# libnxz/power-gzip

Measured on AMD Instinct MI355X. Metric: GiB/s uncompressed in (deflate), real-data corpus in 64 KiB blocks, exact dynamic-Huffman table per block, higher is better.
Workload: dtype u8

## Files before the change

### power-gzip_amd/csrc/nxz_lz77.hip

```cpp
#include <hip/hip_runtime.h>
#include <type_traits>
#include <stdint.h>
#include "nxz_device.h"
#include "nxz_dhtgen_dev.h"
#include "nxz_dict.h"

__device__ unsigned long long *nxz_lz77_prof_buf = nullptr;
#define NXZ_GLOBAL NXZ_GLOBAL_AS
#ifdef NXZ_LZ77_PROF
#define WPROF_BEGIN() unsigned long long wp_ = prof ? clock64() : 0
#define WPROF_END(idx) do { if (prof) { const unsigned long long now_ = clock64(); wacc[(idx) - 16] += now_ - wp_; wp_ = now_; } } while (0)
#define PROF(idx) do { if (prof) { if (t == 0) { unsigned long long now_ = clock64(); profacc[idx] += (uint32_t)(now_ - tprev); tprev = now_; } } } while (0)
#define PCOUNT(idx, n) do { if (prof && lane == 0) atomicAdd(&profacc[idx], (uint32_t)(n)); } while (0)
#ifdef NXZ_LZ77_PROF2
#define PC2(idx, n) do { if (prof && lane == 0) __hip_atomic_fetch_add(&prof[32 + (idx)], (unsigned long long)(n), __ATOMIC_RELAXED, __HIP_MEMORY_SCOPE_AGENT); } while (0)
#else
#define PC2(idx, n) do { } while (0)
#endif
#else
#define PC2(idx, n) do { } while (0)
#define PCOUNT(idx, n) do { } while (0)
#define WPROF_BEGIN() do { } while (0)
#define WPROF_END(idx) do { } while (0)
#define PROF(idx) do { } while (0)
#endif

namespace nxzl77 {

constexpr int NT = 1024;
constexpr int HBITS = 13;
constexpr uint32_t HSIZE = 1u << HBITS;
constexpr uint32_t PTILE = 16384;
constexpr uint32_t PSEG = 16;
constexpr uint32_t NSEG = PTILE / PSEG;
constexpr uint32_t ETILE = 2048;
constexpr uint32_t LAZY_MAX = 32;
constexpr uint32_t MAXMATCH = 258;
constexpr uint32_t WINDOW = 32768;
constexpr uint32_t OPEN2 = 24;
constexpr uint32_t NOHASH = 0xFFFFu;
constexpr uint32_t SECOND_MIN_TOKENS = 3072;
constexpr uint32_t TEXT_HIGH_DIV = 16;
#ifndef NXZ_GROUP_ROUNDS
#define NXZ_GROUP_ROUNDS 24
#endif
#ifndef NXZ_GROUP_MIN
#define NXZ_GROUP_MIN 2
#endif
#ifndef NXZ_GROUP_GATE
#define NXZ_GROUP_GATE 3
#endif
constexpr uint32_t GROUP_ROUNDS = NXZ_GROUP_ROUNDS;
constexpr uint32_t GROUP_GATE = NXZ_GROUP_GATE;
constexpr uint32_t GROUP_MIN = NXZ_GROUP_MIN;
constexpr uint32_t C2_STRIDE = PTILE + 1024;

constexpr uint32_t OFF_IN    = 0;
constexpr uint32_t OFF_HEAD  = 65536 + 32;
constexpr uint32_t OFF_CAND  = OFF_HEAD + HSIZE * 4 + 256;
constexpr uint32_t OFF_MLEN  = OFF_CAND + PTILE * 2;
constexpr uint32_t OFF_SBITS = OFF_MLEN + PTILE;
constexpr uint32_t OFF_MBITS = OFF_SBITS + PTILE / 8;
constexpr uint32_t OFF_X     = OFF_MBITS + PTILE / 8;
constexpr uint32_t OFF_ENTRY = OFF_X + NSEG * 2;
constexpr uint32_t OFF_BITS  = OFF_ENTRY + NSEG * 2;
#ifndef NXZ_LQ_CAP
#define NXZ_LQ_CAP 128
#define NXZ_LQ_MIN 64
#endif
#ifndef NXZ_XQ_CAP
#define NXZ_XQ_CAP 120
#define NXZ_XQ_MIN 56
#endif
constexpr uint32_t LQ_CAP = NXZ_LQ_CAP, LQ_MIN = NXZ_LQ_MIN, XQ_CAP = NXZ_XQ_CAP, XQ_MIN = NXZ_XQ_MIN;
static_assert(LQ_MIN + 64 <= LQ_CAP && XQ_MIN + 64 <= XQ_CAP && LQ_CAP % 8 == 0 && XQ_CAP % 8 == 0, "a batch of 64 must fit behind what waits");
constexpr uint32_t BITS_BYTES = 16 * (LQ_CAP + XQ_CAP) * 2 + 2096 - NSEG * 4 < ETILE * 2 + 64 ? ETILE * 2 + 64 : 16 * (LQ_CAP + XQ_CAP) * 2 + 2096 - NSEG * 4;
constexpr uint32_t OFF_LQ    = OFF_X;
constexpr uint32_t OFF_DQ    = OFF_LQ;
constexpr uint32_t OFF_XQ    = OFF_LQ + 16 * LQ_CAP * 2;
constexpr uint32_t OFF_EB    = OFF_XQ + 16 * XQ_CAP * 2;
constexpr uint32_t EBO       = 32;
static_assert(OFF_EB % 16 == 0 && OFF_EB + 2096 <= OFF_BITS + BITS_BYTES, "match-phase carve");
constexpr uint32_t OFF_SCAN  = OFF_BITS + BITS_BYTES;
constexpr uint32_t OFF_HIST  = OFF_SCAN + 256;
constexpr uint32_t OFF_MISC  = OFF_HIST + 316 * 4;
constexpr uint32_t OFF_PROF  = OFF_MISC + 64;
constexpr uint32_t LDS_BYTES = OFF_PROF + 80;
static_assert(LDS_BYTES <= 163840, "LDS budget");
static_assert(OFF_HEAD % 16 == 0 && OFF_BITS % 16 == 0 && OFF_SCAN % 16 == 0, "alignment");

enum { M_NREC = 0, M_TOK0 = 1, M_HIGH = 2, M_DQ = 3, M_PROGRESS = 4, M_TICKET = 5, M_DEFER = 6, M_NEXT = 7, M_KEEP = 8, M_DEFER2 = 9, M_PREV = 12, M_JOBNO = 13 };
static_assert(M_TICKET == M_PROGRESS + 1 && M_DEFER == M_PROGRESS + 2, "cleared together");

__device__ __forceinline__ uint32_t lds_ld32(const uint32_t *inw, uint32_t r)
{
	uint32_t a = inw[r >> 2], b = inw[(r >> 2) + 1];
	return __builtin_amdgcn_alignbyte(b, a, r & 3);
}

__device__ __forceinline__ uint32_t hash4(uint32_t v) { return (v * 0x9E3779B1u) >> (32 - HBITS); }

__device__ __forceinline__ uint32_t equal16(const uint32_t *inw, uint32_t a, uint32_t b)
{
	const uint32_t aw = a >> 2, bw = b >> 2, as = a & 3, bs = b & 3;
	const uint32_t a0 = inw[aw], a1 = inw[aw + 1], a2 = inw[aw + 2], a3 = inw[aw + 3], a4 = inw[aw + 4];
	const uint32_t b0 = inw[bw], b1 = inw[bw + 1], b2 = inw[bw + 2], b3 = inw[bw + 3], b4 = inw[bw + 4];
	const uint32_t x0 = __builtin_amdgcn_alignbyte(a1, a0, as) ^ __builtin_amdgcn_alignbyte(b1, b0, bs);
	const uint32_t x1 = __builtin_amdgcn_alignbyte(a2, a1, as) ^ __builtin_amdgcn_alignbyte(b2, b1, bs);
	const uint32_t x2 = __builtin_amdgcn_alignbyte(a3, a2, as) ^ __builtin_amdgcn_alignbyte(b3, b2, bs);
	const uint32_t x3 = __builtin_amdgcn_alignbyte(a4, a3, as) ^ __builtin_amdgcn_alignbyte(b4, b3, bs);
	uint32_t n = 16;
	if (x3) n = 12 + ((uint32_t)__builtin_ctz(x3) >> 3);
	if (x2) n = 8 + ((uint32_t)__builtin_ctz(x2) >> 3);
	if (x1) n = 4 + ((uint32_t)__builtin_ctz(x1) >> 3);
	if (x0) n = (uint32_t)__builtin_ctz(x0) >> 3;
	return n;
}

__device__ __forceinline__ uint32_t gf_mul(uint32_t a, uint32_t b)
{
	uint32_t r = 0;
#pragma unroll 8
	for (int i = 0; i < 32; i++) {
		r ^= (b & 0x80000000u) ? a : 0;
// ... 393 lines not shown
					  uint8_t *__restrict__ tokens, uint16_t *__restrict__ cand2,
					  nxz_batch_result_t *__restrict__ results,
					  uint32_t *__restrict__ counts, uint32_t njobs, uint32_t *__restrict__ next_job,
					  const uint8_t *__restrict__ dict)
{
	__shared__ __attribute__((aligned(16))) uint8_t lds[LDS_BYTES];
	uint32_t *inw = (uint32_t *)(lds + OFF_IN);
	uint32_t *head = (uint32_t *)(lds + OFF_HEAD);
	uint16_t *cand = (uint16_t *)(lds + OFF_CAND);
	uint8_t *mlen = lds + OFF_MLEN;
	uint16_t *X = (uint16_t *)(lds + OFF_X);
	uint16_t *entry = (uint16_t *)(lds + OFF_ENTRY);
	uint32_t *sbits = (uint32_t *)(lds + OFF_SBITS);
	uint32_t *mbits = (uint32_t *)(lds + OFF_MBITS);
	uint32_t *tokbits = sbits;
	uint32_t *litbits = mbits;
	uint8_t *mark = lds + OFF_SBITS;
	uint16_t *jump = (uint16_t *)(lds + OFF_MBITS);
	uint32_t *bitbuf = (uint32_t *)(lds + OFF_BITS);
	uint32_t *scan = (uint32_t *)(lds + OFF_SCAN);
	uint32_t *hist = (uint32_t *)(lds + OFF_HIST);
	uint32_t *misc = (uint32_t *)(lds + OFF_MISC);
#ifdef NXZ_LZ77_PROF
	uint32_t *profacc = (uint32_t *)(lds + OFF_PROF);
#endif

#ifdef NXZ_LZ77_PROF
	NXZ_GLOBAL unsigned long long *prof = (NXZ_GLOBAL unsigned long long *)nxz_lz77_prof_buf;
#endif
	if constexpr (GEN) {
		if (threadIdx.x == 0) { misc[M_PREV] = 0; misc[M_JOBNO] = 0; }
		__syncthreads();
	}
	for (uint32_t bid = blockIdx.x; bid < njobs;) {
	if (next_job && threadIdx.x == 0) misc[M_NEXT] = gridDim.x + atomicAdd(next_job, 1u);
	int tid_ = threadIdx.x;
	asm volatile("" : "+v"(tid_));
	const int t = tid_, lane = t & 63, wave = t >> 6;
#ifdef NXZ_LZ77_PROF
	unsigned long long tprev = prof ? clock64() : 0;
	unsigned long long wacc[4] = { 0, 0, 0, 0 };
#endif
	const nxz_batch_job_t job = jobs[bid];
	const uint32_t total = job.src_len;
	const uint32_t h = job.hist_len < total ? job.hist_len : total;
	const uint32_t n = total - h;
	const uint32_t end = total;
	const NXZ_GLOBAL uint8_t *src = (const NXZ_GLOBAL uint8_t *)job.src;
	const uint32_t K1 = n ? (end - 1) >> 6 : 0;
	const uint32_t pw_slice = CRC_POW.v[(1022 - t) & 1023];
	const uint32_t pw_tail = CRC_POW8.v[n ? end - K1 * 64 : 0];

	{
		typedef uint32_t v4u __attribute__((ext_vector_type(4)));
		const NXZ_GLOBAL v4u *s4 = (const NXZ_GLOBAL v4u *)src;
		v4u *d4 = (v4u *)inw;
		uint32_t nfull = total >> 4;
		if constexpr (DICT) {
			const NXZ_GLOBAL v4u *w4 = (const NXZ_GLOBAL v4u *)dict;
			const uint32_t hq = h >> 4;
			for (uint32_t i = t; i < nfull; i += NT) d4[i] = i < hq ? w4[i] : s4[i];
		} else
		for (uint32_t i = t; i < nfull; i += NT) d4[i] = s4[i];
		uint32_t base = nfull << 4;
		for (uint32_t i = base + t; i < base + 48 && i < 65536 + 32; i += NT)
			lds[OFF_IN + i] = i < total ? src[i] : 0;
	}
	for (uint32_t i = t; i < HSIZE; i += NT) head[i] = 0;
	if (t < 316) hist[t] = 0;
	if (t < 16 && t != M_NEXT && !(GEN && (t == M_PREV || t == M_JOBNO))) misc[t] = FUSED && t == M_KEEP ? 3u : 0u;
#ifdef NXZ_LZ77_PROF
	if (t < 20) profacc[t] = 0;
#endif
	{
		uint32_t c = t & 255;
		for (int k = 0; k < 8 * ((t >> 8) + 1); k++) c = (c >> 1) ^ ((c & 1) ? 0xedb88320u : 0);
		bitbuf[t] = c;
	}
	__syncthreads();
	PROF(0);

	uint32_t out_crc, out_adler;
	{
		uint32_t *T = bitbuf;
		const uint32_t initx = job.in_crc ^ 0xffffffffu;
		const int sidx = (int)t - 1023 + (int)K1;
		uint32_t crc = 0, s1 = 0, sj = 0;
		if (n && sidx >= (int)(h >> 6)) {
			const uint4 *sp = (const uint4 *)(lds + OFF_IN + (uint32_t)sidx * 64);
			uint4 q[4] = { sp[0], sp[1], sp[2], sp[3] };
			uint32_t *w = (uint32_t *)q;
			const uint32_t a0 = (uint32_t)sidx * 64;
			if (a0 < h || a0 + 64 > end) {
#pragma unroll
				for (int k = 0; k < 16; k++)
					if (a0 + 4 * k < h || a0 + 4 * k + 4 > end) w[k] = 0;
			}
			uint32_t S = 0, Wt = 0;
#pragma unroll
			for (int k = 0; k < 16; k++) {
				S = __builtin_amdgcn_udot4(w[k], 0x01010101u, S, false);
				Wt = __builtin_amdgcn_udot4(w[k], 0x03020100u + 0x04040404u * k, Wt, false);
			}
			s1 = S;
			sj = S * (n + h - a0) - Wt;
			const uint32_t kfirst = a0 < h ? (h - a0) >> 2 : 0;
			if (a0 <= h && h < a0 + 64) {
				if (h + 4 <= end) {
					if (kfirst == 0) w[0] ^= initx;
					if (kfirst == 4) w[4] ^= initx;
					if (kfirst == 8) w[8] ^= initx;
					if (kfirst == 12) w[12] ^= initx;
				}
			}
			const uint32_t nd = a0 + 64 <= end ? 16 : (end - a0) >> 2;
// ... 9 lines not shown
				uint32_t b0 = v & 0xff, b1 = (v >> 8) & 0xff, b2 = (v >> 16) & 0xff;
				s1 += b0 + b1 + b2;
				sj += (b0 + b1 + b2) * (n - i) - (b1 + 2 * b2);
				if (i == 0) crc ^= initx;
				for (uint32_t k = 0; k < nb; k++) crc = T[(crc ^ (v >> (8 * k))) & 0xff] ^ (crc >> 8);
			}
		}
		uint32_t tailcrc = 0;
		if (t == 1023) { tailcrc = crc; crc = 0; }
		else if (crc) crc = gf_mul(crc, pw_slice);
		for (int o = 32; o > 0; o >>= 1) crc ^= __shfl_down(crc, o, 64);
		if (lane == 0) scan[wave] = crc;
		if (t == 1023) scan[50] = tailcrc;
		uint32_t a1 = s1, a2 = sj % 65521u;
		for (int o = 32; o > 0; o >>= 1) {
			a1 += __shfl_down(a1, o, 64);
			a2 += __shfl_down(a2, o, 64);
		}
		if (lane == 0) { scan[16 + wave] = a1; scan[32 + wave] = a2 % 65521u; }
		__syncthreads();
		if (wave == 0) {
			uint32_t c = lane < 16 ? scan[lane] : 0;
			uint32_t b1 = lane < 16 ? scan[16 + lane] : 0, b2 = lane < 16 ? scan[32 + lane] : 0;
			for (int o = 8; o > 0; o >>= 1) {
				c ^= __shfl_down(c, o, 64);
				b1 += __shfl_down(b1, o, 64);
				b2 += __shfl_down(b2, o, 64);
			}
			if (lane == 0) {
				c = n ? gf_mul(c, pw_tail) ^ scan[50] : initx;
				uint32_t ia = job.in_adler & 0xffff, ib = job.in_adler >> 16;
				uint32_t s1f = (ia + b1) % 65521u;
				uint32_t s2f = (uint32_t)(((uint64_t)ib + (uint64_t)n * ia + b2) % 65521u);
				scan[48] = c ^ 0xffffffffu;
				scan[49] = (s2f << 16) | s1f;
			}
		}
		__syncthreads();
		out_crc = __builtin_amdgcn_readfirstlane(scan[48]);
		out_adler = __builtin_amdgcn_readfirstlane(scan[49]);
		__syncthreads();
	}
	PROF(1);

	if (h) {
		uint32_t *top = (uint32_t *)cand;
		for (uint32_t i = t; i < HSIZE; i += NT) top[i] = 0;
		__syncthreads();
		for (uint32_t r = t; r < h; r += NT)
			if (r + 4 <= end) {
				const uint32_t v = lds_ld32(inw, r);
				const bool deep = r >= 8 && lds_ld32(inw, r - 8) == v && lds_ld32(inw, r - 4) == v && v == __builtin_amdgcn_alignbyte(v, v, 1);
				if (!deep) atomicMax(&top[hash4(v)], r + 1);
			}
		__syncthreads();
		for (uint32_t r = t; r < h; r += NT)
			if (r + 4 <= end) {
				const uint32_t v = lds_ld32(inw, r);
				const bool deep = r >= 8 && lds_ld32(inw, r - 8) == v && lds_ld32(inw, r - 4) == v && v == __builtin_amdgcn_alignbyte(v, v, 1);
				if (!deep && top[hash4(v)] != r + 1) atomicMax(&head[hash4(v)], r + 1);
			}
		__syncthreads();
		for (uint32_t i = t; i < HSIZE; i += NT) head[i] = top[i] | (head[i] << 16);
	}

	NXZ_GLOBAL uint32_t *dstw = (NXZ_GLOBAL uint32_t *)job.dst;
	const uint32_t cap_words = job.dst_cap >> 2;
	uint32_t wordbase = 0, obits = 3;
	const uint32_t gslot = GEN ? (uint32_t)__builtin_amdgcn_readfirstlane((int)misc[M_JOBNO]) & 1u : 0u;
	NXZ_GLOBAL uint8_t *tk = (NXZ_GLOBAL uint8_t *)tokens + (GEN ? ((size_t)blockIdx.x * 2 + gslot) : (size_t)bid) * NXZ_TOK_STRIDE;
	NXZ_GLOBAL uint32_t *g_lit = (NXZ_GLOBAL uint32_t *)(tk + NXZ_TOK_LITBITS);
	NXZ_GLOBAL uint32_t *g_tok = (NXZ_GLOBAL uint32_t *)(tk + NXZ_TOK_MATCHBITS);
	NXZ_GLOBAL uint32_t *g_rec = (NXZ_GLOBAL uint32_t *)(tk + NXZ_TOK_RECORDS);
	NXZ_GLOBAL uint16_t *g_c2 = (NXZ_GLOBAL uint16_t *)cand2 + (size_t)blockIdx.x * C2_STRIDE;
	__syncthreads();

	PROF(2);

	for (uint32_t tb0 = 0; tb0 < n; tb0 += PTILE) {
		const uint32_t tn = n - tb0 < PTILE ? n - tb0 : PTILE;
		const uint32_t nseg = (tn + PSEG - 1) / PSEG;
		const bool hard = __builtin_amdgcn_readfirstlane(misc[M_TOK0]) >= SECOND_MIN_TOKENS;
		const bool text = __builtin_amdgcn_readfirstlane(misc[M_HIGH]) * TEXT_HIGH_DIV < (n < PTILE ? n : PTILE);
		const bool use2 = tb0 == 0 || (hard && !text);
		const uint32_t lazy_max = tb0 != 0 && hard && text ? 0u : LAZY_MAX;
#ifdef NXZ_CHAIN_ALWAYS2
#define CHAIN_USE2 true
#else
#define CHAIN_USE2 use2
#endif

		const uint32_t tnpad = (tn + 511) & ~511u;
		const uint32_t npieces = tnpad >> 9;
		if (t < 3) misc[M_PROGRESS + t] = 0;
		if (t == 3) misc[M_DEFER2] = 0;
		if (t == 4) misc[M_DQ] = 0;
		sbits[t] = 0;
		uint32_t nhigh = 0;
		for (uint32_t piece = wave; piece < npieces; piece += NT / 64) {
#pragma unroll
			for (int it = 0; it < 2; it++) {
				const uint32_t i = (piece << 9) + (it << 8) + 4 * lane, r = h + tb0 + i;
				const uint32_t d0 = inw[r >> 2], d1 = inw[(r >> 2) + 1];
				if (tb0 == 0 && i < tn) nhigh += (uint32_t)__popc(d0 & 0x80808080u);
				const uint32_t v1 = __builtin_amdgcn_alignbyte(d1, d0, 1), v2 = __builtin_amdgcn_alignbyte(d1, d0, 2), v3 = __builtin_amdgcn_alignbyte(d1, d0, 3);
				uint32_t o0 = hash4(d0) << 2, o1 = hash4(v1) << 2, o2 = hash4(v2) << 2, o3 = hash4(v3) << 2;
				const uint32_t dummy = (HSIZE + ((4 * lane) & 63)) * 4;
				if (i + 4 > tn || r + 7 > end) {
					if (i + 0 >= tn || r + 4 > end) o0 = dummy;
					if (i + 1 >= tn || r + 5 > end) o1 = dummy + 4;
					if (i + 2 >= tn || r + 6 > end) o2 = dummy + 8;
					if (i + 3 >= tn || r + 7 > end) o3 = dummy + 12;
				}
				if (r >= 8 && d0 == __builtin_amdgcn_alignbyte(d0, d0, 1) && inw[(r >> 2) - 1] == d0) {
					const uint32_t x2 = inw[(r >> 2) - 2] ^ d0, y = d1 ^ d0;
					if (x2 == 0) o0 = dummy;
					if ((x2 & 0xffffff00u) == 0 && (y & 0xffu) == 0) o1 = dummy + 4;
					if ((x2 & 0xffff0000u) == 0 && (y & 0xffffu) == 0) o2 = dummy + 8;
					if ((x2 & 0xff000000u) == 0 && (y & 0xffffffu) == 0) o3 = dummy + 12;
				}
				*(uint2 *)(cand + i) = make_uint2(o0 | o1 << 16, o2 | o3 << 16);
			}
			__builtin_amdgcn_wave_barrier();
			uint32_t o[8];
#pragma unroll
			for (int u = 0; u < 8; u++) o[u] = cand[(piece << 9) + (u << 6) + lane];
			__builtin_amdgcn_wave_barrier();
			((uint4 *)cand)[(piece << 6) + lane] = make_uint4(o[0] | o[1] << 16, o[2] | o[3] << 16, o[4] | o[5] << 16, o[6] | o[7] << 16);
		}
		if (tb0 == 0) {
			for (int o = 32; o > 0; o >>= 1) nhigh += __shfl_down(nhigh, o, 64);
			if (lane == 0 && nhigh) atomicAdd(&misc[M_HIGH], nhigh);
		}
		{
			uint16_t *eb16 = (uint16_t *)(lds + OFF_EB);
			const uint32_t ngroups = (tn + EBO + 288 + 15) / 16 + 2;
			for (uint32_t g = t; g < ngroups; g += NT) {
				const int32_t r0s = (int32_t)(h + tb0 + 16 * g) - (int32_t)EBO;
				const uint32_t r0 = r0s < 0 ? end : (uint32_t)r0s;
				uint32_t bits = 0;
				if (r0 < end) {
					const uint4 dv = *(const uint4 *)(lds + OFF_IN + r0);
					const uint32_t pv = r0 ? inw[(r0 >> 2) - 1] : 0;
					auto eq4 = [](uint32_t d, uint32_t prev) -> uint32_t {
						const uint32_t xx = d ^ __builtin_amdgcn_alignbyte(d, prev, 3);
						const uint32_t nzb = (((xx & 0x7f7f7f7fu) + 0x7f7f7f7fu) | xx) & 0x80808080u;
						return ~((((nzb >> 7) * 0x00204081u) >> 21)) & 0xf;
					};
					bits = eq4(dv.x, pv) | eq4(dv.y, dv.x) << 4 | eq4(dv.z, dv.y) << 8 | eq4(dv.w, dv.z) << 12;
					if (r0 == 0) bits &= ~1u;
					if (end - r0 < 16) bits &= (1u << (end - r0)) - 1;
				}
				eb16[g] = (uint16_t)bits;
			}
		}
		__syncthreads();
		PROF(3);

		if (wave == 0) {
			uint8_t *headb = (uint8_t *)head;
			__builtin_amdgcn_s_setprio(3);
			int clane = lane;
			asm volatile("" : "+v"(clane));
			auto unpack = [](const uint4 pk, uint32_t (&off)[8]) {
				off[0] = pk.x & 0xffff; off[1] = pk.x >> 16; off[2] = pk.y & 0xffff; off[3] = pk.y >> 16;
				off[4] = pk.z & 0xffff; off[5] = pk.z >> 16; off[6] = pk.w & 0xffff; off[7] = pk.w >> 16;
			};
			auto steps = [&](const uint4 pk, uint32_t piece, uint32_t (&old)[8]) {
				uint32_t off[8]; unpack(pk, off);
#pragma unroll
				for (int u = 0; u < 8; u++) {
					uint32_t *slot = (uint32_t *)(headb + off[u]);
					old[u] = __hip_atomic_load(slot, __ATOMIC_RELAXED, __HIP_MEMORY_SCOPE_WORKGROUP);
					__builtin_amdgcn_wave_barrier();
					*(uint16_t *)slot = (uint16_t)(h + tb0 + (piece << 9) + 64 * u + clane + 1);
					__builtin_amdgcn_wave_barrier();
				}
			};
			auto note = [&](const uint4 pk, const uint32_t (&old)[8]) {
				if (!CHAIN_USE2) return;
				uint32_t off[8]; unpack(pk, off);
#pragma unroll
				for (int u = 0; u < 8; u++) *(uint16_t *)(headb + off[u] + 2) = (uint16_t)old[u];
				__builtin_amdgcn_wave_barrier();
			};
			auto hand = [&](const uint32_t (&o)[8], uint32_t piece) {
				typedef uint32_t v4u __attribute__((ext_vector_type(4)));
#pragma unroll
				for (int u = 0; u < 8; u++) cand[(piece << 9) + 64 * u + lane] = (uint16_t)o[u];
				if (CHAIN_USE2) {
					((NXZ_GLOBAL v4u *)g_c2)[(piece << 6) + lane] = (v4u){ __builtin_amdgcn_perm(o[1], o[0], 0x07060302), __builtin_amdgcn_perm(o[3], o[2], 0x07060302),
											    __builtin_amdgcn_perm(o[5], o[4], 0x07060302), __builtin_amdgcn_perm(o[7], o[6], 0x07060302) };
					__builtin_amdgcn_wave_barrier();
					__builtin_amdgcn_s_waitcnt(0x0F71);
				}
				__builtin_amdgcn_wave_barrier();
				if (lane == 0) __hip_atomic_store(&misc[M_PROGRESS], piece, __ATOMIC_RELAXED, __HIP_MEMORY_SCOPE_WORKGROUP);
				__builtin_amdgcn_wave_barrier();
			};
			const uint32_t dm = (HSIZE + lane) * 4 | ((HSIZE + lane) * 4) << 16;
			const uint4 dummy = make_uint4(dm, dm, dm, dm);
			uint4 pkB = dummy;
			uint32_t oA[8], oB[8];
			for (uint32_t base = 0; base < npieces; base += 2) {
				const uint4 *cp = (const uint4 *)cand + (base << 6) + lane;
				const bool two = base + 1 < npieces;
				const uint4 l1 = cp[two ? 64 : 0];
				const uint4 pkA = cp[0];
				steps(pkA, base, oA);
				if (base) { note(pkB, oB); hand(oB, base - 1); }
				pkB = two ? l1 : dummy;
				steps(pkB, base + 1, oB);
				note(pkA, oA);
				hand(oA, base);
			}
			{
				const uint32_t lastp = ((npieces + 1) & ~1u) - 1;
				note(pkB, oB);
				hand(oB, lastp);
				__builtin_amdgcn_s_waitcnt(0x0F70);
				__builtin_amdgcn_wave_barrier();
				if (lane == 0) __hip_atomic_store(&misc[M_PROGRESS], npieces, __ATOMIC_RELAXED, __HIP_MEMORY_SCOPE_WORKGROUP);
			}
			__builtin_amdgcn_s_setprio(0);
		}
		PROF(4);

		auto first_zero = [](const uint32_t *bm, uint32_t s0, uint32_t limit) -> uint32_t {
			uint32_t wi = (s0 >> 5) & ~3u;
			uint4 q = *(const uint4 *)(bm + wi);
			const uint32_t sw = (s0 >> 5) & 3, lowmask = ~(~0u << (s0 & 31));
			uint32_t w0 = ~q.x, w1 = ~q.y, w2 = ~q.z, w3 = ~q.w;
			if (sw > 0) w0 = 0; if (sw > 1) w1 = 0; if (sw > 2) w2 = 0;
			if (sw == 0) w0 &= ~lowmask; else if (sw == 1) w1 &= ~lowmask; else if (sw == 2) w2 &= ~lowmask; else w3 &= ~lowmask;
			for (;;) {
				if (w0 | w1 | w2 | w3) {
					const uint32_t pos = wi * 32 + (w0 ? (uint32_t)__builtin_ctz(w0) : w1 ? 32 + (uint32_t)__builtin_ctz(w1)
								  : w2 ? 64 + (uint32_t)__builtin_ctz(w2) : 96 + (uint32_t)__builtin_ctz(w3));
					return pos < limit ? pos : limit;
				}
				wi += 4;
				if (wi * 32 >= limit) return limit;
				q = *(const uint4 *)(bm + wi);
				w0 = ~q.x; w1 = ~q.y; w2 = ~q.z; w3 = ~q.w;
			}
		};
		uint32_t *kb = mbits;
		uint32_t *vb = sbits;
		{
			const uint32_t *eb = (const uint32_t *)(lds + OFF_EB);
			auto bits32 = [](const uint32_t *bm, uint32_t b) -> uint32_t {
				const uint32_t lo = bm[b >> 5], hi = bm[(b >> 5) + 1], sh = b & 31;
				return sh ? (lo >> sh) | (hi << (32 - sh)) : lo;
			};
			uint16_t *lq = (uint16_t *)(lds + OFF_LQ) + wave * LQ_CAP;
// ... 150 lines not shown
					}
					const unsigned long long ml = __ballot(open);
					if (ml) {
						if (open) xq[xqn + __popcll(ml & ((1ull << lane) - 1))] = (uint16_t)i;
						xqn += (uint32_t)__popcll(ml);
						PCOUNT(14, __popcll(ml));
						__builtin_amdgcn_wave_barrier();
					}
					pb &= pb - 1;
					const bool more = __ballot(pb != 0) != 0;
					if (xqn >= XQ_MIN || (last && !more && nq <= 64 && xqn)) { level2(xqn); xqn = 0; }
					if (!more) break;
				} while (true);
			};
			const uint32_t nunits = (tn + 255) >> 8;
			for (;;) {
				uint32_t unit = 0;
				if (lane == 0) unit = atomicAdd(&misc[M_TICKET], 1u);
				unit = __builtin_amdgcn_readfirstlane(unit);
				const bool last = unit >= nunits;
				const uint32_t piece = unit >> 1;
				uint32_t qbits = 0;
				const uint32_t it = unit & 1;
				const uint32_t ib = unit << 8;
				const uint32_t i4 = ib + 4 * lane, r4 = h + tb0 + i4;
				WPROF_BEGIN();
				if (!last) {
					while (__hip_atomic_load(&misc[M_PROGRESS], __ATOMIC_RELAXED, __HIP_MEMORY_SCOPE_WORKGROUP) <= piece)
						__builtin_amdgcn_s_sleep(4);
					__builtin_amdgcn_fence(__ATOMIC_ACQUIRE, "workgroup");
					WPROF_END(16);
					auto quad = [&](auto fullt, auto use2t) {
						constexpr bool FULL = decltype(fullt)::value, USE2 = decltype(use2t)::value;
						uint32_t q2[4] = { 0, 0, 0, 0 };
						if constexpr (USE2) {
#pragma unroll
							for (int j = 0; j < 4; j++)
								q2[j] = __hip_atomic_load(g_c2 + (piece << 9) + (4 * (lane & 15) + j) * 8 + 4 * it + (lane >> 4), __ATOMIC_RELAXED, __HIP_MEMORY_SCOPE_AGENT);
						}
						const uint2 qq = *(const uint2 *)(cand + i4);
						const uint32_t w14 = bits32(eb, EBO + i4 - 7);
						const uint32_t d0 = inw[r4 >> 2], d1 = inw[(r4 >> 2) + 1], d2 = inw[(r4 >> 2) + 2];
						uint32_t mw = 0, c01 = 0, c23 = 0, vbits = 0, kbits = 0;
						bool okA[4], raw8[4], lng[4];
						uint32_t dA[4];
#pragma unroll
						for (int j = 0; j < 4; j++) {
							const uint32_t i = i4 + j, r = r4 + j;
							const bool ok = (FULL || (i < tn && r + 4 <= end)) && ((w14 >> j) & 0x7ff) != 0x7ff;
							const uint32_t maxlen = FULL || end - r >= MAXMATCH ? MAXMATCH : end - r;
							const uint32_t v = j ? __builtin_amdgcn_alignbyte(d1, d0, j) : d0, v4 = j ? __builtin_amdgcn_alignbyte(d2, d1, j) : d1;
							auto probe = [&](uint32_t entry, uint32_t &dist1) -> uint32_t {
								const uint32_t qc = (uint16_t)(entry - 1);
								dist1 = r - qc - 1;
								const bool qok = ok && dist1 < WINDOW;
								const uint32_t q = FULL || qok ? qc : 0;
								const uint32_t qa = q >> 2, u0 = inw[qa], u1 = inw[qa + 1], u2 = inw[qa + 2];
								const uint32_t qv = __builtin_amdgcn_alignbyte(u1, u0, q & 3), qv4 = __builtin_amdgcn_alignbyte(u2, u1, q & 3);
								const uint32_t x = qv4 ^ v4;
								uint32_t n8 = 4 + ((x ? (uint32_t)__builtin_ctz(x) : 32u) >> 3);
								if (!FULL && n8 > maxlen) n8 = maxlen;
								return qok && qv == v ? n8 : 0;
							};
							uint32_t d1st, d2nd;
							const uint32_t n1st = probe((j & 2 ? qq.y : qq.x) >> (16 * (j & 1)), d1st);
							uint32_t n2nd = 0;
							d2nd = 0;
							if constexpr (USE2) n2nd = probe(q2[j], d2nd);
							const bool second = n2nd > n1st;
							const uint32_t lenA = second ? n2nd : n1st;
							okA[j] = lenA != 0;
							dA[j] = second ? d2nd : d1st;
							raw8[j] = lenA == 8;
// ... 291 lines not shown
					}
					break;
				}
				const uint32_t rest = (seg_nz | vis1) >> k;
				uint32_t run = rest ? (uint32_t)__builtin_ctz(rest) : 16 - k;
				if (run > lim - p) run = lim - p;
				if (run) {
					lm |= ((1u << run) - 1) << k;
					p += run;
					continue;
				}
				bool m;
				const uint32_t l = seg_step(p, lim, m);
				lm |= (m ? 0u : 1u) << k;
				mm |= (m ? 1u : 0u) << k;
				if (m) mlen[p] = (uint8_t)(l - 3);
				p += l;
			}
			const uint32_t sh = 16 * ((uint32_t)t & 1), wi = (uint32_t)t >> 1;
			const uint64_t lv = (uint64_t)lm << sh, mv = (uint64_t)mm << sh;
			if ((uint32_t)lv) atomicOr(&litbits[wi], (uint32_t)lv);
			if (lv >> 32) atomicOr(&litbits[wi + 1], (uint32_t)(lv >> 32));
			if ((uint32_t)mv) atomicOr(&tokbits[wi], (uint32_t)mv);
			if (mv >> 32) atomicOr(&tokbits[wi + 1], (uint32_t)(mv >> 32));
		}
		__syncthreads();
		PROF(8);
		if (tb0 == 0 && n > PTILE && t < 512) {
			uint32_t c = (uint32_t)__popc(litbits[t]) + (uint32_t)__popc(tokbits[t]);
			for (int o = 32; o > 0; o >>= 1) c += __shfl_down(c, o, 64);
			if (lane == 0) atomicAdd(&misc[M_TOK0], c);
		}

		if constexpr (FUSED) {
			Quad q[4] = { {0, 0, 0, 0}, {0, 0, 0, 0}, {0, 0, 0, 0}, {0, 0, 0, 0} };
			uint32_t nb = 0;
			if (p0 < tn) {
				const uint32_t tok16 = ((const uint16_t *)tokbits)[t], lit16 = ((const uint16_t *)litbits)[t];
				if (tok16 | lit16) {
					const uint4 bv = *(const uint4 *)(lds + OFF_IN + h + tb0 + p0);
					const uint4 mv = *(const uint4 *)(mlen + p0);
					const uint4 c0 = ((const uint4 *)cand)[2 * t], c1 = ((const uint4 *)cand)[2 * t + 1];
					q[0] = fx_quad(bv.x, lit16 & 15, tok16 & 15, mv.x, c0.x, c0.y);
					q[1] = fx_quad(bv.y, (lit16 >> 4) & 15, (tok16 >> 4) & 15, mv.y, c0.z, c0.w);
					q[2] = fx_quad(bv.z, (lit16 >> 8) & 15, (tok16 >> 8) & 15, mv.z, c1.x, c1.y);
					q[3] = fx_quad(bv.w, lit16 >> 12, tok16 >> 12, mv.w, c1.z, c1.w);
					nb = q[0].nb + q[1].nb + q[2].nb + q[3].nb;
				}
			}
			const uint32_t incl = wave_incl_scan(nb, lane);
			if (lane == 63) scan[wave] = incl;
			__syncthreads();
			uint32_t bitpos = obits + incl - nb, tilebits = 0;
#pragma unroll
			for (int w = 0; w < 16; w++) {
				const uint32_t sc = scan[w];
				if (w < wave) bitpos += sc;
				tilebits += sc;
			}
			uint32_t *win = (uint32_t *)(lds + OFF_CAND);
			const uint32_t tot = obits + tilebits, nfull = tot >> 5;
			for (uint32_t i = t; i < (nfull + 8) / 4 + 1; i += NT) ((uint4 *)win)[i] = make_uint4(0, 0, 0, 0);
			__syncthreads();
			if (t == 0) atomicOr(&win[0], misc[M_KEEP]);
			fx_emit(win, q[0], bitpos);
			fx_emit(win, q[1], bitpos + q[0].nb);
			fx_emit(win, q[2], bitpos + q[0].nb + q[1].nb);
			fx_emit(win, q[3], bitpos + q[0].nb + q[1].nb + q[2].nb);
			__syncthreads();
			for (uint32_t i = t; i < nfull; i += NT)
				if (wordbase + i < cap_words) dstw[wordbase + i] = win[i];
			if (t == 0) misc[M_KEEP] = win[nfull];
			wordbase += nfull;
			obits = tot & 31;
			__syncthreads();
		} else
		{
			const uint32_t tok16 = p0 < tn ? ((const uint16_t *)tokbits)[t] : 0;
			const uint32_t nm = (uint32_t)__popc(tok16);
			uint32_t incl = wave_incl_scan(nm, lane);
			if (lane == 63) scan[wave] = incl;
			const uint32_t recbase = misc[M_NREC];
			__syncthreads();
			uint32_t rank = recbase + incl - nm, tot = 0;
#pragma unroll
			for (int w = 0; w < 16; w++) {
				const uint32_t sc = scan[w];
				if (w < wave) rank += sc;
				tot += sc;
			}
			for (uint32_t mbits_ = tok16; mbits_; mbits_ &= mbits_ - 1) {
				const uint32_t p = p0 + (uint32_t)__builtin_ctz(mbits_);
				const uint32_t l3 = mlen[p], d = cand[p];
				if (rank < NXZ_TOK_MAXREC) g_rec[rank] = l3 | (d << 8);
				rank++;
				if (COUNT) {
					uint32_t le = l3 < 8 ? 0 : (29 - (uint32_t)__builtin_clz(l3 | 8));
					const uint32_t ls = l3 == 255 ? 28 : (le << 2) + (l3 >> le);
					const uint32_t de = d < 4 ? 0 : (30 - (uint32_t)__builtin_clz(d | 4));
					const uint32_t ds = d < 4 ? d : 2 * de + 2 + ((d >> de) & 1);
					atomicAdd(&hist[257 + ls], 1u);
					atomicAdd(&hist[286 + ds], 1u);
				}
			}
			if (COUNT && p0 < tn) {
				const uint32_t lit16 = ((const uint16_t *)litbits)[t];
				if (lit16) {
					const uint4 bv = *(const uint4 *)(lds + OFF_IN + h + tb0 + p0);
					for (uint32_t lb = lit16; lb; lb &= lb - 1) {
						const uint32_t k = (uint32_t)__builtin_ctz(lb);
						const uint32_t a = (k & 8) ? bv.z : bv.x, b = (k & 8) ? bv.w : bv.y;
						const uint32_t w = (k & 4) ? b : a;
						atomicAdd(&hist[(w >> (8 * (k & 3))) & 0xff], 1u);
					}
				}
			}
			{
				const uint32_t nwords = (tn + 31) >> 5, i = (uint32_t)t & 511;
				if (i < nwords) {
					if (t < 512) g_lit[(tb0 >> 5) + i] = litbits[i];
					else g_tok[(tb0 >> 5) + i] = tokbits[i];
				}
			}
			__syncthreads();
			if (t == 0) misc[M_NREC] = recbase + tot;
		}
		PROF(9);
	}

	if (t == 0) {
		nxz_batch_result_t r;
		r.cc = 0; r.tpbc = 0; r.tebc = 0;
		r.spbc = DICT ? n : total; r.crc = out_crc; r.adler = out_adler; r.subc = 0;
		r.sfbt = misc[M_NREC];
		if constexpr (FUSED) {
			const uint64_t acc = misc[M_KEEP];
			const uint32_t bits = obits + 7;
			const uint64_t totbits = (uint64_t)wordbase * 32 + bits;
			const uint32_t tpbc = (uint32_t)((totbits + 7) >> 3);
			uint32_t cc = wordbase > cap_words || tpbc > job.dst_cap ? NXZ_CC_TARGET_SPACE : 0;
			if (!cc) {
				NXZ_GLOBAL uint8_t *o = (NXZ_GLOBAL uint8_t *)job.dst + (size_t)wordbase * 4;
				for (uint32_t b = 0; b < (bits + 7) / 8; b++) o[b] = (uint8_t)(acc >> (8 * b));
				if (tpbc > total) cc = NXZ_CC_TPBC_GT_SPBC;
			}
			r.cc = cc; r.tpbc = cc == NXZ_CC_TARGET_SPACE ? 0 : tpbc; r.tebc = (uint32_t)(totbits & 7); r.sfbt = 0;
		}
		results[bid] = r;
	}
#ifdef NXZ_LZ77_PROF
	if (prof) {
		if (lane == 0) for (int k = 0; k < 4; k++) atomicAdd(&profacc[16 + k], (uint32_t)wacc[k]);
		__syncthreads();
		if (t < 20) __hip_atomic_fetch_add(&prof[t], (unsigned long long)profacc[t], __ATOMIC_RELAXED, __HIP_MEMORY_SCOPE_AGENT);
	}
#endif
	if (COUNT && (!GEN || counts)) {
		__syncthreads();
		if (t < 316) counts[(size_t)bid * 316 + t] = (t == 256) ? 1u : hist[t];
	}
	if constexpr (GEN) {
		__builtin_amdgcn_fence(__ATOMIC_RELEASE, "workgroup");
		__syncthreads();
		__builtin_amdgcn_fence(__ATOMIC_ACQUIRE, "workgroup");
		const uint32_t prev = (uint32_t)__builtin_amdgcn_readfirstlane((int)misc[M_PREV]);
		gen::post(lds, jobs, (NXZ_GLOBAL uint8_t *)tokens, results, true, gslot, prev, gslot ^ 1u, t);
		if (t == 0) { misc[M_PREV] = bid + 1; misc[M_JOBNO] = misc[M_JOBNO] + 1; }
	}
	__syncthreads();
	const uint32_t drawn = next_job ? misc[M_NEXT] : bid + gridDim.x;
	__syncthreads();
	bid = drawn;
	}
	if constexpr (GEN) {
		const uint32_t prev = (uint32_t)__builtin_amdgcn_readfirstlane((int)misc[M_PREV]);
		const uint32_t slot = ((uint32_t)__builtin_amdgcn_readfirstlane((int)misc[M_JOBNO]) & 1u) ^ 1u;
		if (prev) gen::post(lds, jobs, (NXZ_GLOBAL uint8_t *)tokens, results, false, 0, prev, slot, (int)threadIdx.x);
	}
}

template <bool COUNT, bool FUSED = false, bool GEN = false>
__global__ __launch_bounds__(NT) void lz77_kernel(const nxz_batch_job_t *__restrict__ jobs,
						  uint8_t *__restrict__ tokens, uint16_t *__restrict__ cand2,
						  nxz_batch_result_t *__restrict__ results,
						  uint32_t *__restrict__ counts, uint32_t njobs, uint32_t *__restrict__ next_job)
{
	lz77_body<COUNT, FUSED, GEN, false>(jobs, tokens, cand2, results, counts, njobs, next_job, nullptr);
}

template <bool COUNT, bool FUSED = false, bool GEN = false>
__global__ __launch_bounds__(NT) void lz77_dict_kernel(const nxz_batch_job_t *__restrict__ jobs,
						       uint8_t *__restrict__ tokens, uint16_t *__restrict__ cand2,
						       nxz_batch_result_t *__restrict__ results,
						       uint32_t *__restrict__ counts, uint32_t njobs, uint32_t *__restrict__ next_job,
						       const uint8_t *__restrict__ dict)
{
	lz77_body<COUNT, FUSED, GEN, true>(jobs, tokens, cand2, results, counts, njobs, next_job, dict);
}

__global__ __launch_bounds__(256) void dict_jobs_kernel(const nxz_batch_job_t *__restrict__ in, uint32_t n, uint32_t W, nxz_batch_job_t *__restrict__ out)
{
	const uint32_t i = blockIdx.x * 256 + threadIdx.x;
	if (i >= n) return;
	nxz_batch_job_t j = in[i];
	if (nxz_dict_job_fits(W, j.src_len, j.hist_len)) {
// ... 84 lines not shown
```

Before: 102.3.

## Prefetch next job's leading input into hash-head LDS during final tile

```diff
diff --git a/power-gzip_amd/csrc/nxz_lz77.hip b/power-gzip_amd/csrc/nxz_lz77.hip
--- a/power-gzip_amd/csrc/nxz_lz77.hip
+++ b/power-gzip_amd/csrc/nxz_lz77.hip
@@ -89,7 +89,7 @@
 static_assert(LDS_BYTES <= 163840, "LDS budget");
 static_assert(OFF_HEAD % 16 == 0 && OFF_BITS % 16 == 0 && OFF_SCAN % 16 == 0, "alignment");
 
-enum { M_NREC = 0, M_TOK0 = 1, M_HIGH = 2, M_DQ = 3, M_PROGRESS = 4, M_TICKET = 5, M_DEFER = 6, M_NEXT = 7, M_KEEP = 8, M_DEFER2 = 9, M_PREV = 12, M_JOBNO = 13 };
+enum { M_NREC = 0, M_TOK0 = 1, M_HIGH = 2, M_DQ = 3, M_PROGRESS = 4, M_TICKET = 5, M_DEFER = 6, M_NEXT = 7, M_KEEP = 8, M_DEFER2 = 9, M_CRC = 10, M_ADLER = 11, M_PREV = 12, M_JOBNO = 13 };
 static_assert(M_TICKET == M_PROGRESS + 1 && M_DEFER == M_PROGRESS + 2, "cleared together");
 
 __device__ __forceinline__ uint32_t lds_ld32(const uint32_t *inw, uint32_t r)
@@ -549,6 +549,7 @@
 		if (threadIdx.x == 0) { misc[M_PREV] = 0; misc[M_JOBNO] = 0; }
 		__syncthreads();
 	}
+	bool prefetched = false;
 	for (uint32_t bid = blockIdx.x; bid < njobs;) {
 	if (next_job && threadIdx.x == 0) misc[M_NEXT] = gridDim.x + atomicAdd(next_job, 1u);
 	int tid_ = threadIdx.x;
@@ -571,19 +572,31 @@
 	{
 		typedef uint32_t v4u __attribute__((ext_vector_type(4)));
 		const NXZ_GLOBAL v4u *s4 = (const NXZ_GLOBAL v4u *)src;
-		v4u *d4 = (v4u *)inw;
+		v4u *d4 = (v4u *)inw, *h4 = (v4u *)head;
 		uint32_t nfull = total >> 4;
-		if constexpr (DICT) {
-			const NXZ_GLOBAL v4u *w4 = (const NXZ_GLOBAL v4u *)dict;
-			const uint32_t hq = h >> 4;
-			for (uint32_t i = t; i < nfull; i += NT) d4[i] = i < hq ? w4[i] : s4[i];
-		} else
-		for (uint32_t i = t; i < nfull; i += NT) d4[i] = s4[i];
+		const NXZ_GLOBAL v4u *w4 = (const NXZ_GLOBAL v4u *)dict;
+		const uint32_t hq = DICT ? h >> 4 : 0;
+		static_assert(HSIZE * 4 == 2 * NT * 16, "two quads a lane clear head[]");
+		uint32_t zero_ = 0;
+		asm volatile("" : "+v"(zero_));
+		const v4u z4 = { zero_, zero_, zero_, zero_ };
+#pragma unroll
+		for (int half = 1; half >= 0; half--) {
+			const uint32_t i0 = (uint32_t)t + NT * 2 * half, i1 = i0 + NT;
+			v4u q0 = z4, q1 = z4;
+			if (half == 0 && prefetched) { q0 = h4[i0]; q1 = h4[i1]; }
+			else {
+				if (i0 < nfull) q0 = DICT && i0 < hq ? w4[i0] : s4[i0];
+				if (i1 < nfull) q1 = DICT && i1 < hq ? w4[i1] : s4[i1];
+			}
+			if (half == 0) { h4[i0] = z4; h4[i1] = z4; }
+			if (i0 < nfull) d4[i0] = q0;
+			if (i1 < nfull) d4[i1] = q1;
+		}
 		uint32_t base = nfull << 4;
 		for (uint32_t i = base + t; i < base + 48 && i < 65536 + 32; i += NT)
 			lds[OFF_IN + i] = i < total ? src[i] : 0;
 	}
-	for (uint32_t i = t; i < HSIZE; i += NT) head[i] = 0;
 	if (t < 316) hist[t] = 0;
 	if (t < 16 && t != M_NEXT && !(GEN && (t == M_PREV || t == M_JOBNO))) misc[t] = FUSED && t == M_KEEP ? 3u : 0u;
 #ifdef NXZ_LZ77_PROF
@@ -597,7 +610,6 @@
 	__syncthreads();
 	PROF(0);
 
-	uint32_t out_crc, out_adler;
 	{
 		uint32_t *T = bitbuf;
 		const uint32_t initx = job.in_crc ^ 0xffffffffu;
@@ -673,14 +685,10 @@
 				uint32_t ia = job.in_adler & 0xffff, ib = job.in_adler >> 16;
 				uint32_t s1f = (ia + b1) % 65521u;
 				uint32_t s2f = (uint32_t)(((uint64_t)ib + (uint64_t)n * ia + b2) % 65521u);
-				scan[48] = c ^ 0xffffffffu;
-				scan[49] = (s2f << 16) | s1f;
-			}
-		}
-		__syncthreads();
-		out_crc = __builtin_amdgcn_readfirstlane(scan[48]);
-		out_adler = __builtin_amdgcn_readfirstlane(scan[49]);
-		__syncthreads();
+				misc[M_CRC] = c ^ 0xffffffffu;
+				misc[M_ADLER] = (s2f << 16) | s1f;
+			}
+		}
 	}
 	PROF(1);
 
@@ -718,6 +726,7 @@
 
 	PROF(2);
 
+	bool prefetched_next = false;
 	for (uint32_t tb0 = 0; tb0 < n; tb0 += PTILE) {
 		const uint32_t tn = n - tb0 < PTILE ? n - tb0 : PTILE;
 		const uint32_t nseg = (tn + PSEG - 1) / PSEG;
@@ -1442,6 +1451,29 @@
 			if (lane == 0) atomicAdd(&misc[M_TOK0], c);
 		}
 
+		typedef uint32_t v4u __attribute__((ext_vector_type(4)));
+		uint32_t zero_ = 0;
+		asm volatile("" : "+v"(zero_));
+		v4u nx0 = { zero_, zero_, zero_, zero_ }, nx1 = nx0;
+		bool park = false;
+		uint32_t nq = 0;
+		if constexpr (!GEN) {
+			if (tb0 + PTILE >= n) {
+				const uint32_t nb = (uint32_t)__builtin_amdgcn_readfirstlane((int)(next_job ? misc[M_NEXT] : bid + gridDim.x));
+				if (nb < njobs) {
+					const uint32_t ntotal = jobs[nb].src_len, nhist = jobs[nb].hist_len;
+					const NXZ_GLOBAL v4u *s4 = (const NXZ_GLOBAL v4u *)jobs[nb].src;
+					const NXZ_GLOBAL v4u *w4 = (const NXZ_GLOBAL v4u *)dict;
+					nq = ntotal >> 4;
+					const uint32_t hq = DICT ? (nhist < ntotal ? nhist : ntotal) >> 4 : 0;
+					if ((uint32_t)t < nq) nx0 = DICT && (uint32_t)t < hq ? w4[t] : s4[t];
+					if ((uint32_t)t + NT < nq) nx1 = DICT && (uint32_t)t + NT < hq ? w4[t + NT] : s4[t + NT];
+					park = true;
+				}
+			}
+		}
+		prefetched_next = park;
+
 		if constexpr (FUSED) {
 			Quad q[4] = { {0, 0, 0, 0}, {0, 0, 0, 0}, {0, 0, 0, 0}, {0, 0, 0, 0} };
 			uint32_t nb = 0;
@@ -1478,6 +1510,8 @@
 			fx_emit(win, q[2], bitpos + q[0].nb + q[1].nb);
 			fx_emit(win, q[3], bitpos + q[0].nb + q[1].nb + q[2].nb);
 			__syncthreads();
+			if ((uint32_t)t < nq) ((v4u *)head)[t] = nx0;
+			if ((uint32_t)t + NT < nq) ((v4u *)head)[t + NT] = nx1;
 			for (uint32_t i = t; i < nfull; i += NT)
 				if (wordbase + i < cap_words) dstw[wordbase + i] = win[i];
 			if (t == 0) misc[M_KEEP] = win[nfull];
@@ -1532,6 +1566,8 @@
 					else g_tok[(tb0 >> 5) + i] = tokbits[i];
 				}
 			}
+			if ((uint32_t)t < nq) ((v4u *)head)[t] = nx0;
+			if ((uint32_t)t + NT < nq) ((v4u *)head)[t + NT] = nx1;
 			__syncthreads();
 			if (t == 0) misc[M_NREC] = recbase + tot;
 		}
@@ -1541,7 +1577,7 @@
 	if (t == 0) {
 		nxz_batch_result_t r;
 		r.cc = 0; r.tpbc = 0; r.tebc = 0;
-		r.spbc = DICT ? n : total; r.crc = out_crc; r.adler = out_adler; r.subc = 0;
+		r.spbc = DICT ? n : total; r.crc = misc[M_CRC]; r.adler = misc[M_ADLER]; r.subc = 0;
 		r.sfbt = misc[M_NREC];
 		if constexpr (FUSED) {
 			const uint64_t acc = misc[M_KEEP];
@@ -1581,6 +1617,7 @@
 	const uint32_t drawn = next_job ? misc[M_NEXT] : bid + gridDim.x;
 	__syncthreads();
 	bid = drawn;
+	prefetched = prefetched_next;
 	}
 	if constexpr (GEN) {
 		const uint32_t prev = (uint32_t)__builtin_amdgcn_readfirstlane((int)misc[M_PREV]);
```

Measured after the change: 101.2. -1.1%, worse.

## Split chain handoff into local progress and global ring flags, transpose candidate layout

Applied to the files above, without the earlier changes.

```diff
diff --git a/power-gzip_amd/csrc/nxz_lz77.hip b/power-gzip_amd/csrc/nxz_lz77.hip
--- a/power-gzip_amd/csrc/nxz_lz77.hip
+++ b/power-gzip_amd/csrc/nxz_lz77.hip
@@ -12,6 +12,11 @@
 #define WPROF_END(idx) do { if (prof) { const unsigned long long now_ = clock64(); wacc[(idx) - 16] += now_ - wp_; wp_ = now_; } } while (0)
 #define PROF(idx) do { if (prof) { if (t == 0) { unsigned long long now_ = clock64(); profacc[idx] += (uint32_t)(now_ - tprev); tprev = now_; } } } while (0)
 #define PCOUNT(idx, n) do { if (prof && lane == 0) atomicAdd(&profacc[idx], (uint32_t)(n)); } while (0)
+#ifdef NXZ_LZ77_PROF_CHAIN
+#define CPROF(k) do { if (prof) { const unsigned long long now_ = clock64(); cacc[k] += now_ - cp_; cp_ = now_; } } while (0)
+#else
+#define CPROF(k) do { } while (0)
+#endif
 #ifdef NXZ_LZ77_PROF2
 #define PC2(idx, n) do { if (prof && lane == 0) __hip_atomic_fetch_add(&prof[32 + (idx)], (unsigned long long)(n), __ATOMIC_RELAXED, __HIP_MEMORY_SCOPE_AGENT); } while (0)
 #else
@@ -23,6 +28,7 @@
 #define WPROF_BEGIN() do { } while (0)
 #define WPROF_END(idx) do { } while (0)
 #define PROF(idx) do { } while (0)
+#define CPROF(k) do { } while (0)
 #endif
 
 namespace nxzl77 {
@@ -85,11 +91,11 @@
 constexpr uint32_t OFF_HIST  = OFF_SCAN + 256;
 constexpr uint32_t OFF_MISC  = OFF_HIST + 316 * 4;
 constexpr uint32_t OFF_PROF  = OFF_MISC + 64;
-constexpr uint32_t LDS_BYTES = OFF_PROF + 80;
+constexpr uint32_t LDS_BYTES = OFF_PROF + 96;
 static_assert(LDS_BYTES <= 163840, "LDS budget");
 static_assert(OFF_HEAD % 16 == 0 && OFF_BITS % 16 == 0 && OFF_SCAN % 16 == 0, "alignment");
 
-enum { M_NREC = 0, M_TOK0 = 1, M_HIGH = 2, M_DQ = 3, M_PROGRESS = 4, M_TICKET = 5, M_DEFER = 6, M_NEXT = 7, M_KEEP = 8, M_DEFER2 = 9, M_PREV = 12, M_JOBNO = 13 };
+enum { M_NREC = 0, M_TOK0 = 1, M_HIGH = 2, M_DQ = 3, M_PROGRESS = 4, M_TICKET = 5, M_DEFER = 6, M_NEXT = 7, M_KEEP = 8, M_DEFER2 = 9, M_RING = 10, M_PREV = 12, M_JOBNO = 13 };
 static_assert(M_TICKET == M_PROGRESS + 1 && M_DEFER == M_PROGRESS + 2, "cleared together");
 
 __device__ __forceinline__ uint32_t lds_ld32(const uint32_t *inw, uint32_t r)
@@ -557,6 +563,7 @@
 #ifdef NXZ_LZ77_PROF
 	unsigned long long tprev = prof ? clock64() : 0;
 	unsigned long long wacc[4] = { 0, 0, 0, 0 };
+	unsigned long long cacc[4] = { 0, 0, 0, 0 }, cp_ = 0;
 #endif
 	const nxz_batch_job_t job = jobs[bid];
 	const uint32_t total = job.src_len;
@@ -587,7 +594,7 @@
 	if (t < 316) hist[t] = 0;
 	if (t < 16 && t != M_NEXT && !(GEN && (t == M_PREV || t == M_JOBNO))) misc[t] = FUSED && t == M_KEEP ? 3u : 0u;
 #ifdef NXZ_LZ77_PROF
-	if (t < 20) profacc[t] = 0;
+	if (t < 24) profacc[t] = 0;
 #endif
 	{
 		uint32_t c = t & 255;
@@ -736,6 +743,7 @@
 		if (t < 3) misc[M_PROGRESS + t] = 0;
 		if (t == 3) misc[M_DEFER2] = 0;
 		if (t == 4) misc[M_DQ] = 0;
+		if (t == 5) misc[M_RING] = 0;
 		sbits[t] = 0;
 		uint32_t nhigh = 0;
 		for (uint32_t piece = wave; piece < npieces; piece += NT / 64) {
@@ -801,6 +809,9 @@
 		if (wave == 0) {
 			uint8_t *headb = (uint8_t *)head;
 			__builtin_amdgcn_s_setprio(3);
+#ifdef NXZ_LZ77_PROF_CHAIN
+			if (prof) cp_ = clock64();
+#endif
 			int clane = lane;
 			asm volatile("" : "+v"(clane));
 			auto unpack = [](const uint4 pk, uint32_t (&off)[8]) {
@@ -817,6 +828,7 @@
 					*(uint16_t *)slot = (uint16_t)(h + tb0 + (piece << 9) + 64 * u + clane + 1);
 					__builtin_amdgcn_wave_barrier();
 				}
+				CPROF(0);
 			};
 			auto note = [&](const uint4 pk, const uint32_t (&old)[8]) {
 				if (!CHAIN_USE2) return;
@@ -824,20 +836,49 @@
 #pragma unroll
 				for (int u = 0; u < 8; u++) *(uint16_t *)(headb + off[u] + 2) = (uint16_t)old[u];
 				__builtin_amdgcn_wave_barrier();
+				CPROF(1);
 			};
 			auto hand = [&](const uint32_t (&o)[8], uint32_t piece) {
 				typedef uint32_t v4u __attribute__((ext_vector_type(4)));
+#ifdef NXZ_HAND_NATURAL
 #pragma unroll
 				for (int u = 0; u < 8; u++) cand[(piece << 9) + 64 * u + lane] = (uint16_t)o[u];
+#else
+				{
+					uint2 *hp = (uint2 *)(cand + (piece << 9)) + clane;
+					hp[0] = make_uint2(__builtin_amdgcn_perm(o[1], o[0], 0x05040100), __builtin_amdgcn_perm(o[3], o[2], 0x05040100));
+					hp[64] = make_uint2(__builtin_amdgcn_perm(o[5], o[4], 0x05040100), __builtin_amdgcn_perm(o[7], o[6], 0x05040100));
+				}
+#endif
+				if (CHAIN_USE2)
+					((NXZ_GLOBAL v4u *)g_c2)[(piece << 6) + clane] = (v4u){ __builtin_amdgcn_perm(o[1], o[0], 0x07060302), __builtin_amdgcn_perm(o[3], o[2], 0x07060302),
+											    __builtin_amdgcn_perm(o[5], o[4], 0x07060302), __builtin_amdgcn_perm(o[7], o[6], 0x07060302) };
+#ifdef NXZ_RING_ONE_WORD
+				CPROF(2);
 				if (CHAIN_USE2) {
-					((NXZ_GLOBAL v4u *)g_c2)[(piece << 6) + lane] = (v4u){ __builtin_amdgcn_perm(o[1], o[0], 0x07060302), __builtin_amdgcn_perm(o[3], o[2], 0x07060302),
-											    __builtin_amdgcn_perm(o[5], o[4], 0x07060302), __builtin_amdgcn_perm(o[7], o[6], 0x07060302) };
 					__builtin_amdgcn_wave_barrier();
 					__builtin_amdgcn_s_waitcnt(0x0F71);
 				}
+				CPROF(3);
 				__builtin_amdgcn_wave_barrier();
-				if (lane == 0) __hip_atomic_store(&misc[M_PROGRESS], piece, __ATOMIC_RELAXED, __HIP_MEMORY_SCOPE_WORKGROUP);
+				if (lane == 0) {
+					__hip_atomic_store(&misc[M_PROGRESS], piece, __ATOMIC_RELAXED, __HIP_MEMORY_SCOPE_WORKGROUP);
+					__hip_atomic_store(&misc[M_RING], piece, __ATOMIC_RELAXED, __HIP_MEMORY_SCOPE_WORKGROUP);
+				}
 				__builtin_amdgcn_wave_barrier();
+#else
+				__builtin_amdgcn_wave_barrier();
+				if (lane == 0) __hip_atomic_store(&misc[M_PROGRESS], piece + 1, __ATOMIC_RELAXED, __HIP_MEMORY_SCOPE_WORKGROUP);
+				CPROF(2);
+				if (CHAIN_USE2) {
+					__builtin_amdgcn_wave_barrier();
+					__builtin_amdgcn_s_waitcnt(0x0F72);
+					CPROF(3);
+					__builtin_amdgcn_wave_barrier();
+					if (lane == 0 && piece >= 2) __hip_atomic_store(&misc[M_RING], piece - 1, __ATOMIC_RELAXED, __HIP_MEMORY_SCOPE_WORKGROUP);
+				}
+				__builtin_amdgcn_wave_barrier();
+#endif
 			};
 			const uint32_t dm = (HSIZE + lane) * 4 | ((HSIZE + lane) * 4) << 16;
 			const uint4 dummy = make_uint4(dm, dm, dm, dm);
@@ -861,7 +902,11 @@
 				hand(oB, lastp);
 				__builtin_amdgcn_s_waitcnt(0x0F70);
 				__builtin_amdgcn_wave_barrier();
-				if (lane == 0) __hip_atomic_store(&misc[M_PROGRESS], npieces, __ATOMIC_RELAXED, __HIP_MEMORY_SCOPE_WORKGROUP);
+				if (lane == 0) {
+					__hip_atomic_store(&misc[M_PROGRESS], lastp + 1, __ATOMIC_RELAXED, __HIP_MEMORY_SCOPE_WORKGROUP);
+					__hip_atomic_store(&misc[M_RING], lastp + 1, __ATOMIC_RELAXED, __HIP_MEMORY_SCOPE_WORKGROUP);
+				}
+				CPROF(3);
 			}
 			__builtin_amdgcn_s_setprio(0);
 		}
@@ -1078,13 +1123,24 @@
 					WPROF_END(16);
 					auto quad = [&](auto fullt, auto use2t) {
 						constexpr bool FULL = decltype(fullt)::value, USE2 = decltype(use2t)::value;
+						int mlane = lane;
+						asm volatile("" : "+v"(mlane));
+						const uint32_t tq = 16 * ((uint32_t)mlane & 15) + ((uint32_t)mlane >> 4);
+#ifdef NXZ_HAND_NATURAL
+						const uint2 qq = *(const uint2 *)(cand + i4);
+#else
+						const uint16_t *cq = cand + ib + tq;
+						const uint2 qq = make_uint2((uint32_t)cq[0] | (uint32_t)cq[4] << 16, (uint32_t)cq[8] | (uint32_t)cq[12] << 16);
+#endif
 						uint32_t q2[4] = { 0, 0, 0, 0 };
 						if constexpr (USE2) {
+							while (__hip_atomic_load(&misc[M_RING], __ATOMIC_RELAXED, __HIP_MEMORY_SCOPE_WORKGROUP) <= piece)
+								__builtin_amdgcn_s_sleep(2);
+							WPROF_END(16);
 #pragma unroll
 							for (int j = 0; j < 4; j++)
-								q2[j] = __hip_atomic_load(g_c2 + (piece << 9) + (4 * (lane & 15) + j) * 8 + 4 * it + (lane >> 4), __ATOMIC_RELAXED, __HIP_MEMORY_SCOPE_AGENT);
+								q2[j] = __hip_atomic_load(g_c2 + (piece << 9) + 2 * tq - ((uint32_t)mlane >> 4) + 8 * j + 4 * it, __ATOMIC_RELAXED, __HIP_MEMORY_SCOPE_AGENT);
 						}
-						const uint2 qq = *(const uint2 *)(cand + i4);
 						const uint32_t w14 = bits32(eb, EBO + i4 - 7);
 						const uint32_t d0 = inw[r4 >> 2], d1 = inw[(r4 >> 2) + 1], d2 = inw[(r4 >> 2) + 2];
 						uint32_t mw = 0, c01 = 0, c23 = 0, vbits = 0, kbits = 0;
@@ -1561,8 +1617,9 @@
 #ifdef NXZ_LZ77_PROF
 	if (prof) {
 		if (lane == 0) for (int k = 0; k < 4; k++) atomicAdd(&profacc[16 + k], (uint32_t)wacc[k]);
-		__syncthreads();
-		if (t < 20) __hip_atomic_fetch_add(&prof[t], (unsigned long long)profacc[t], __ATOMIC_RELAXED, __HIP_MEMORY_SCOPE_AGENT);
+		if (t == 0) for (int k = 0; k < 4; k++) profacc[20 + k] += (uint32_t)cacc[k];
+		__syncthreads();
+		if (t < 24) __hip_atomic_fetch_add(&prof[t], (unsigned long long)profacc[t], __ATOMIC_RELAXED, __HIP_MEMORY_SCOPE_AGENT);
 	}
 #endif
 	if (COUNT && (!GEN || counts)) {
```

After: 102.4 before, 103.2 after (median of 6 runs). Within noise of the previous version (+0.8%).
